# alexklwong/calibrated-backprojection-network

Hardware: AMD Instinct MI355X
Metric: depth-completion frames/sec at 352x1216 (higher is better)
Workload: dtype f32; 1 GPU; KITTI 352x1216, batch 32/GPU, fp32, full KBNet forward in HIP, random xavier weights; frames_per_gpu=32, global_batch=32, height=352, width=1216, n_ranks_seen=1, collective_backend=nccl, gathered_frames=32, launch=HIP graph replay, 2 concurrent sub-batch branch(es)

## Files before the change

### calibrated-backprojection-network_amd/csrc/conv_split.hip

```cpp
#include "conv_common.h"

#ifndef KBN_SPLIT_STRAIGHT
#define KBN_SPLIT_STRAIGHT 1
#endif
#ifndef KBN_SPLIT_PRIO
#define KBN_SPLIT_PRIO 0
#endif

namespace kbn {

typedef _Float16 sph8 __attribute__((ext_vector_type(8)));
typedef _Float16 sph2 __attribute__((ext_vector_type(2)));
typedef float spf16 __attribute__((ext_vector_type(16)));
typedef float spf4 __attribute__((ext_vector_type(4)));
typedef _Float16 sph4 __attribute__((ext_vector_type(4)));

constexpr int SP_TW = 32, SP_CK = 16, SP_MB = 4, SP_TH = 16, SP_THREADS = 512;
constexpr int SP_WEXP = 13;

template <int MODE>
struct SpGeom {
    static constexpr bool UP = MODE == 1, S2 = MODE == 2;
    static constexpr int TH = S2 ? 8 : SP_TH;
    static constexpr int ROWS = UP ? TH / 2 + 2 : (S2 ? 2 * TH + 1 : TH + 2);
    static constexpr int COLS = UP ? SP_TW / 2 + 2 : (S2 ? 2 * SP_TW + 1 : SP_TW + 2), NPIX = ROWS * COLS;
    static constexpr int A_PART = 2 * NPIX * 16, A_BYTES = 2 * A_PART;
    static constexpr int LDS = 2 * A_BYTES;
    static constexpr int PR = (NPIX + 255) / 256;
    static constexpr int NLOADA = PR * 8;
};

struct SplitConvParams {
    const float* src[2];
    long long src_bstride[2];
    int srcC[2];
    int nsrc;
    const float* inv_scale;
    const _Float16* wp;
    float* out;
    long long out_bstride;
    int N, OC, Cin, H, W;
    int sH, sW;
    int tilesX, tilesY, nTilesN, nblocks;
    int act;
    float slope;
    int vec4;
    float prescale;
    float unscale;
    const unsigned* amax[2];
    unsigned* out_amax;
    const _Float16* pair_src;
    long long pair_src_bstride;
    const float* pair_src_scale;
    _Float16* pair_out;
    long long pair_out_bstride;
    float* pair_out_scale;
    const float* l1;
    int tp_x0, tp_tilesY, tp_nblocks;
    int sub0;
    const float* xyz;
    long long xyz_bstride;
    const float* wxyz;
    int ksplit;
    long long ks_stride;
};

__device__ __forceinline__ void sp_split8(const float (&v)[8], float prescale, sph8& h1, sph8& h2) {
    const float prescale_hi = prescale * 2048.f;
#pragma unroll
    for (int k = 0; k < 8; k += 2) {
        const f32x2 a = {v[k], v[k + 1]};
        const sph2 c1 = __builtin_convertvector(a * prescale, sph2);
        const f32x2 f = {(float)c1[0], (float)c1[1]};
        const f32x2 hi = a * prescale_hi;
        const f32x2 r = {__builtin_fmaf(f[0], -2048.f, hi[0]), __builtin_fmaf(f[1], -2048.f, hi[1])};
        const sph2 c2 = __builtin_convertvector(r, sph2);
        h1[k] = c1[0]; h1[k + 1] = c1[1];
        h2[k] = c2[0]; h2[k + 1] = c2[1];
    }
}

__device__ __forceinline__ void sp_act_scale(const SplitConvParams& p, int n, float& prescale, float& unscale) {
    prescale = p.prescale;
    unscale = p.unscale;
    if (p.amax[0]) {
        unsigned b = p.amax[0][n];
        if (p.amax[1]) b = max(b, p.amax[1][n]);
        int k = 14 + 127 - (int)(b >> 23);
        k = k > 100 ? 100 : (k < -100 ? -100 : k);
        prescale = __uint_as_float((unsigned)(127 + k) << 23);
        unscale = __uint_as_float((unsigned)(127 - k) << 23);
    }
}
__device__ __forceinline__ float sp_amax4(float m, const f32x4& v) {
    return fmaxf(fmaxf(m, fmaxf(fin_abs(v[0]), fin_abs(v[1]))), fmaxf(fin_abs(v[2]), fin_abs(v[3])));
}


__device__ __forceinline__ float sp_scale_of_bound(float bound) {
    int k = 14 + 127 - (int)(__float_as_uint(bound) >> 23 & 255u);
    k = k > 100 ? 100 : (k < -100 ? -100 : k);
    return __uint_as_float((unsigned)(127 + k) << 23);
}
__device__ __forceinline__ float sp_pair_out_scale(const SplitConvParams& p, int n) {
    const int nchunks = p.Cin / SP_CK, n0 = p.nsrc > 1 ? p.srcC[0] / SP_CK : nchunks;
    float w0 = 0.f, w1 = 0.f;
    for (int c = 0; c < n0; ++c) w0 += p.l1[c];
    for (int c = n0; c < nchunks; ++c) w1 += p.l1[c];
    float bound = __uint_as_float(p.amax[0][n]) * w0;
    if (p.nsrc > 1) bound += __uint_as_float(p.amax[1][n]) * w1;
    return sp_scale_of_bound(bound);
}
__device__ __forceinline__ void sp_act_scale_of(const SplitConvParams& p, int s, int n, float& prescale, float& unscale) {
// ... 56 lines not shown
__global__ void pack_split_kernel(const float* __restrict__ w, const float* __restrict__ inv_scale, _Float16* __restrict__ packed,
                                  int OC, int Cin, int nchunks, int NT, long long total, int taps, int skip_at, int skip) {
    const long long e = (long long)blockIdx.x * blockDim.x + threadIdx.x;
    if (e >= total) return;
    const int per_chunk = taps * 2 * 2 * NT * 8;
    int r = (int)(e % per_chunk);
    const long long q = e / per_chunk;
    const int chunk = (int)(q % nchunks), nt = (int)(q / nchunks);
    const int tap = r / (2 * 2 * NT * 8); r -= tap * 2 * 2 * NT * 8;
    const int part = r / (2 * NT * 8); r -= part * 2 * NT * 8;
    const int g = r / (NT * 8); r -= g * NT * 8;
    const int n = r >> 3, k = r & 7;
    const int c = chunk * SP_CK + g * 8 + k, oc = nt * NT + n;
    _Float16 h = (_Float16)0.f;
    if (c < Cin && oc < OC) {
        const int cw = c < skip_at ? c : c + skip;
        const float ws = w[((long long)oc * (Cin + skip) + cw) * taps + tap] * (1.f / inv_scale[oc]);
        const _Float16 w1 = (_Float16)ws;
        h = part == 0 ? w1 : (_Float16)((ws - (float)w1) * 2048.f);

    }
    packed[e] = h;
}

__global__ __launch_bounds__(256) void split_l1_kernel(const float* __restrict__ w, float* __restrict__ l1, int OC, int Cin, int taps) {
    __shared__ float red[256];
    const int c = blockIdx.x;
    float m = 0.f;
    for (int oc = threadIdx.x; oc < OC; oc += 256) {
        const float* wp = w + ((long long)oc * Cin + c * SP_CK) * taps;
        float sum = 0.f;
        for (int e = 0; e < SP_CK * taps; ++e) sum += fabsf(wp[e]);
        m = fmaxf(m, sum);
    }
    red[threadIdx.x] = m;
    __syncthreads();
    for (int st = 128; st > 0; st >>= 1) {
        if ((int)threadIdx.x < st) red[threadIdx.x] = fmaxf(red[threadIdx.x], red[threadIdx.x + st]);
        __syncthreads();
    }
    if (threadIdx.x == 0) l1[c] = red[0];
}

template <bool VEC>
__global__ __launch_bounds__(256) void absmax_frames_kernel(const float* __restrict__ x, long long batch_stride, long long per_frame,
                                                            unsigned* __restrict__ slots) {
    const float* xn = x + (long long)blockIdx.y * batch_stride;
    float m = 0.f;
    const long long stride = (long long)gridDim.x * 256;
    if constexpr (VEC) {
        const f32x4* x4 = reinterpret_cast<const f32x4*>(xn);
        const long long n4 = per_frame >> 2;
        long long i = (long long)blockIdx.x * 256 + threadIdx.x;
        for (; i + 3 * stride < n4; i += 4 * stride) {
            const f32x4 a = x4[i], b = x4[i + stride], c = x4[i + 2 * stride], d = x4[i + 3 * stride];
            m = sp_amax4(sp_amax4(sp_amax4(sp_amax4(m, a), b), c), d);
        }
        for (; i < n4; i += stride) m = sp_amax4(m, x4[i]);
        for (long long t = (n4 << 2) + (long long)blockIdx.x * 256 + threadIdx.x; t < per_frame; t += stride) m = fmaxf(m, fin_abs(xn[t]));
    } else {
        for (long long i = (long long)blockIdx.x * 256 + threadIdx.x; i < per_frame; i += stride) m = fmaxf(m, fin_abs(xn[i]));
    }
    absmax_commit(slots + blockIdx.y, m);
}

int absmax_frames_launch(const float* x, long long batch_stride, int n, long long per_frame, unsigned* slots, hipStream_t stream) {
    if (!x || !slots || n < 1 || per_frame < 1) return KBN_ERR_INVALID_ARGUMENT;
    const bool vec = !((reinterpret_cast<uintptr_t>(x) & 15) || (batch_stride & 3));
    const int blocks = (int)std::min<long long>(std::max(1, 2048 / n), (per_frame + 4095) / 4096);
    if (vec) hipLaunchKernelGGL(absmax_frames_kernel<true>, dim3(blocks, n), dim3(256), 0, stream, x, batch_stride, per_frame, slots);
    else hipLaunchKernelGGL(absmax_frames_kernel<false>, dim3(blocks, n), dim3(256), 0, stream, x, batch_stride, per_frame, slots);
    KBN_CHECK_LAUNCH();
    return KBN_OK;
}

template <int N, int NBX>
__device__ __forceinline__ void sp_wait_b(f32x4 (&b)[NBX][2]) {
    static_assert(NBX == 1 || NBX == 2, "one or two 32-filter blocks per wave");
    if constexpr (NBX == 2) asm volatile("s_waitcnt vmcnt(%4)" : "+v"(b[0][0]), "+v"(b[0][1]), "+v"(b[1][0]), "+v"(b[1][1]) : "n"(N));
    else asm volatile("s_waitcnt vmcnt(%2)" : "+v"(b[0][0]), "+v"(b[0][1]) : "n"(N));
}

template <int MODE, int RG, bool APART, bool BLDS, int NBW = 2, bool PIN0 = false, bool POUT = false, bool MIXED = false, bool ONE = false, bool KSPLIT = false>
__global__ __launch_bounds__(SP_THREADS, 1) void conv3x3_split_kernel(const SplitConvParams p) {
    static_assert(!MIXED || (MODE == 0 && BLDS), "transposed tiles: the concat kernel");
    extern __shared__ __attribute__((aligned(16))) unsigned char smem[];
    if (!MIXED || (int)blockIdx.x < p.nblocks) {
        constexpr bool TP = false;
        const int block = blockIdx.x, nblocks = p.nblocks, tilesX = p.tilesX, tilesY = p.tilesY;
#include "conv_split_body.inc"
    } else if constexpr (MIXED) {
        constexpr bool TP = true;
        const int block = (int)blockIdx.x - p.nblocks, nblocks = p.tp_nblocks, tilesX = 1, tilesY = p.tp_tilesY;
#include "conv_split_body.inc"
    }
}

constexpr int UF_NT = 32, UF_ITEMS = 16;
struct UfItem { int ox, s, py, dy, px, dx; };
__host__ __device__ constexpr UfItem uf_item(int it) {
    int ox = it < 4 ? 0 : (it < 12 ? 1 : 2);
    int r = it - (ox == 0 ? 0 : (ox == 1 ? 4 : 12));
    const int ncol = ox == 1 ? 2 : 1;
    const int rowidx = r / ncol, colidx = r % ncol;
    const int s = rowidx == 0 ? 0 : (rowidx < 3 ? 1 : 2);
    const int py = s == 0 ? 0 : (s == 2 ? 1 : rowidx - 1);
    const int px = ox == 0 ? 0 : (ox == 2 ? 1 : colidx);
    return UfItem{ox, s, py, s - py, px, ox - px};
}
__device__ __forceinline__ void uf_taps(int p, int d, int tr, int& k0, int& k1) {
    if (tr) { k0 = p == 0 ? 1 : (d == 0 ? 2 : 0); k1 = (p == 0 && d == 0) ? 0 : k0; return; }
    k0 = (p == 0) ? (d == 0 ? 0 : 1) : (d == 0 ? 0 : 2);
    k1 = (p == 0) ? (d == 0 ? 0 : 2) : (d == 0 ? 1 : 2);
}
__device__ __forceinline__ float uf_fold(const float* w9, int py, int dy, int px, int dx, int tr = 0) {
    int r0, r1, c0, c1;
    uf_taps(py, dy, tr, r0, r1);
    uf_taps(px, dx, tr, c0, c1);
    float acc = 0.f;
    for (int r = r0; r <= r1; ++r) {
        float row = 0.f;
        for (int c = c0; c <= c1; ++c) row += w9[r * 3 + c];
        acc += row;
    }
    return acc;
}

__global__ void uf_scale_kernel(const float* __restrict__ w, float* __restrict__ inv_scale, int OC, int Cin, int tr) {
    const int oc = blockIdx.x;
    __shared__ float red[256];
    float m = 0.f;
    if (oc < OC)
        for (int i = threadIdx.x; i < Cin * UF_ITEMS; i += 256) {
            const int c = i / UF_ITEMS;
            const UfItem t = uf_item(i % UF_ITEMS);
            m = fmaxf(m, fabsf(uf_fold(w + ((long long)oc * Cin + c) * 9, t.py, t.dy, t.px, t.dx, tr)));
        }
    red[threadIdx.x] = m;
    __syncthreads();
    for (int s = 128; s > 0; s >>= 1) {
        if (threadIdx.x < s) red[threadIdx.x] = fmaxf(red[threadIdx.x], red[threadIdx.x + s]);
        __syncthreads();
    }
    if (threadIdx.x == 0) {
        int ex = SP_WEXP;
        if (red[0] > 0.f && red[0] < 3.0e38f) (void)frexpf(red[0], &ex);
        int e = SP_WEXP - ex;
        e = e > 100 ? 100 : (e < -100 ? -100 : e);
        inv_scale[oc] = ldexpf(1.f, -e);
    }
}

__global__ void uf_pack_kernel(const float* __restrict__ w, const float* __restrict__ inv_scale, _Float16* __restrict__ packed,
                               int OC, int Cin, int nchunks, long long total, int tr) {
    const long long e = (long long)blockIdx.x * blockDim.x + threadIdx.x;
    if (e >= total) return;
    constexpr int per_item = 2 * 2 * UF_NT * 8, per_chunk = UF_ITEMS * per_item;
    int r = (int)(e % per_chunk);
    const long long q = e / per_chunk;
    const int chunk = (int)(q % nchunks), nt = (int)(q / nchunks);
    const int item = r / per_item; r -= item * per_item;
    const int part = r / (2 * UF_NT * 8); r -= part * 2 * UF_NT * 8;
    const int g = r / (UF_NT * 8); r -= g * UF_NT * 8;
    const int n = r >> 3, k = r & 7;
    const int c = chunk * SP_CK + g * 8 + k, oc = nt * UF_NT + n;
    _Float16 h = (_Float16)0.f;
    if (c < Cin && oc < OC) {
// ... 944 lines not shown
            if (s != 0 || mode == 1) return KBN_ERR_UNSUPPORTED;
            if (mode == 2 && n_src != 1) return KBN_ERR_UNSUPPORTED;
            if (mode == 0 && (n_src != 2 || a.channels < 2 * SP_CK || srcs[1].kind != KBN_SRC_TENSOR || srcs[1].channels < 2 * SP_CK))
                return KBN_ERR_UNSUPPORTED;
            if (!a.scale || (reinterpret_cast<uintptr_t>(a.data) & 15) || (a.batch_stride & 7) ||
                a.batch_stride < (long long)(a.channels / 8) * 2 * pair_plane_halves(a.src_height, a.src_width))
                return KBN_ERR_INVALID_ARGUMENT;
            if ((long long)a.src_height * a.src_width >= 0x0fffffffLL) return KBN_ERR_UNSUPPORTED;
            p.pair_src = reinterpret_cast<const _Float16*>(a.data); p.pair_src_bstride = a.batch_stride; p.pair_src_scale = a.scale;
        } else {
            p.src[s] = a.data; p.src_bstride[s] = a.batch_stride;
        }
        p.srcC[s] = a.channels;
        cin += a.channels;
    }
    if (p.pair_src && !p.src[0]) { p.src[0] = p.src[1]; p.src_bstride[0] = p.src_bstride[1]; }
    const bool dims_ok = mode == 0 ? (p.sH == height && p.sW == width)
                       : mode != 2 ? (2 * p.sH == height && 2 * p.sW == width)
                                   : (ceil_div(p.sH, 2) == height && ceil_div(p.sW, 2) == width);
    if (!dims_ok) return KBN_ERR_INVALID_ARGUMENT;
    if ((long long)p.sH * p.sW > 0x1fffffffLL || (long long)height * width > 0x1fffffffLL) return KBN_ERR_UNSUPPORTED;
    if (n_src == 1) { p.src[1] = p.src[0]; p.src_bstride[1] = p.src_bstride[0]; p.srcC[1] = 0; }
    p.nsrc = n_src;
    if (srcs[0].absmax && (n_src == 1 || srcs[1].absmax)) { p.amax[0] = srcs[0].absmax; p.amax[1] = n_src > 1 ? srcs[1].absmax : nullptr; }
    else if (p.pair_src && n_src > 1 && srcs[1].absmax) p.amax[1] = srcs[1].absmax;
    p.out_amax = out_absmax;
    const int ntf = split_nt(mode, out_channels, cin);
    p.nTilesN = ceil_div(out_channels, ntf);
    p.inv_scale = static_cast<const float*>(packed_weight);
    p.wp = reinterpret_cast<const _Float16*>(p.inv_scale + p.nTilesN * ntf);
    p.l1 = reinterpret_cast<const float*>(static_cast<const unsigned char*>(packed_weight) +
                                          kbn_conv3x3_split_packed_weight_bytes(out_channels, cin, mode) - (size_t)(cin / SP_CK) * 4);
    if (pair_out) {
        const bool narrow = mode == 3 && uf_narrow(out_channels, cin) && !(knob(KNOB_DEBUG) & 128);
        const bool kernel_ok = (mode == 0) || (mode == 3 && ntf == U64_NT && !uf_narrow(out_channels, cin)) ||
                               (mode == 2 && n_src == 1) || narrow;
        if (!kernel_ok || (!narrow && (out_channels & 7))) return KBN_ERR_UNSUPPORTED;
        const int pair_channels = narrow ? U16_NT : out_channels;
        if (!p.amax[0] || (n_src > 1 && !p.amax[1]) || !pair_out_scale || (reinterpret_cast<uintptr_t>(pair_out) & 15) ||
            (pair_out_batch_stride & 7) || pair_out_batch_stride < (long long)(pair_channels / 8) * 2 * pair_plane_halves(height, width))
            return KBN_ERR_INVALID_ARGUMENT;
        p.pair_out = static_cast<_Float16*>(pair_out); p.pair_out_bstride = pair_out_batch_stride; p.pair_out_scale = pair_out_scale;
    }
    if (p.pair_src && mode == 3 && !(ntf == U64_NT || uf_narrow(out_channels, cin))) return KBN_ERR_UNSUPPORTED;
    if (p.pair_src && mode == 3 && uf_narrow(out_channels, cin) && (srcs[0].channels % U16_CK)) return KBN_ERR_UNSUPPORTED;
    p.out = out; p.out_bstride = out_batch_stride;
    p.N = n; p.OC = out_channels; p.Cin = cin; p.H = height; p.W = width;
    p.tilesX = ceil_div(width, SP_TW); p.tilesY = ceil_div(height, mode == 2 ? SpGeom<2>::TH : SpGeom<0>::TH);
    if (mode == 3) { p.tilesX = ceil_div(p.sW, 32); p.tilesY = ceil_div(p.sH, 16); }
    const long long blocks = (long long)p.tilesX * p.tilesY * n * p.nTilesN;
    if (blocks > 0x7fffffffLL) return KBN_ERR_UNSUPPORTED;
    p.nblocks = (int)blocks;
    p.act = apply_activation ? 1 : 0; p.slope = negative_slope;
    p.prescale = ldexpf(1.f, act_exponent); p.unscale = ldexpf(1.f, -act_exponent);
    p.vec4 = vec4 ? 1 : 0;
    p.ksplit = 1;
    if (ksplit > 1) {
        const bool up64 = mode == 3 && ntf == U64_NT && !uf_narrow(out_channels, cin);
        if ((mode != 0 && mode != 2 && !up64) || p.pair_src || pair_out || !workspace || !out || knob(KNOB_FP16_ONE_TERM)) return KBN_ERR_UNSUPPORTED;
        const int nchunks = cin / SP_CK;
        if (ksplit > nchunks || (long long)(ceil_div(nchunks, ksplit)) * (ksplit - 1) >= nchunks) return KBN_ERR_INVALID_ARGUMENT;
        if (blocks * ksplit > 0x7fffffffLL) return KBN_ERR_UNSUPPORTED;
        const long long per_frame = (long long)out_channels * height * width;
        SplitConvParams q = p;
        q.ksplit = ksplit;
        q.out = workspace; q.out_bstride = per_frame; q.ks_stride = per_frame * n;
        q.out_amax = nullptr; q.act = 0;
        q.vec4 = !((width & 3) || (reinterpret_cast<uintptr_t>(workspace) & 15)) ? 1 : 0;
        q.nblocks = (int)(blocks * ksplit);
        static DeviceOnce ok0, ok2, ok3;
        if (up64) {
            q.tilesX = ceil_div(p.sW, 32); q.tilesY = ceil_div(p.sH, 8);
            const long long b64 = (long long)q.tilesX * q.tilesY * n * p.nTilesN * ksplit;
            if (b64 > 0x7fffffffLL) return KBN_ERR_UNSUPPORTED;
            q.nblocks = (int)b64;
            auto kern = upconv2x_split64_kernel<false, false, false, false, true>;
            if (int r = set_max_dynamic_lds(ok3, reinterpret_cast<const void*>(kern), 160 * 1024)) return r;
            hipLaunchKernelGGL(kern, dim3(q.nblocks), dim3(SP_THREADS), 2 * (2 * 2 * 10 * 34 * 16) + 2 * (8 * 2 * 2 * 64 * 16), (hipStream_t)stream, q);
        } else if (mode == 0) {
            auto kern = conv3x3_split_kernel<0, 8, true, true, 2, false, false, false, false, true>;
            if (int r = set_max_dynamic_lds(ok0, reinterpret_cast<const void*>(kern), 160 * 1024)) return r;
            hipLaunchKernelGGL(kern, dim3(q.nblocks), dim3(SP_THREADS), SpGeom<0>::LDS + 2 * 9 * 2 * 2 * 64 * 16, (hipStream_t)stream, q);
        } else {
            auto kern = conv3x3_split_kernel<2, 2, true, false, 1, false, false, false, false, true>;
            if (int r = set_max_dynamic_lds(ok2, reinterpret_cast<const void*>(kern), 160 * 1024)) return r;
            hipLaunchKernelGGL(kern, dim3(q.nblocks), dim3(SP_THREADS), SpGeom<2>::LDS, (hipStream_t)stream, q);
        }
        KBN_CHECK_LAUNCH();
        const float slope = apply_activation ? negative_slope : 1.f;
        const bool vec = !(per_frame & 3) && !(out_batch_stride & 3) && !((reinterpret_cast<uintptr_t>(out) | reinterpret_cast<uintptr_t>(workspace)) & 15);
        const long long items = vec ? per_frame / 4 : per_frame;
        long long kr = items / (256LL * 512);
        kr = kr < 1 ? 1 : (kr > 8 ? 8 : kr);
        const dim3 grid((unsigned)((items + 256 * kr - 1) / (256 * kr)), (unsigned)n);
        if (vec) hipLaunchKernelGGL(ksplit_reduce_kernel<true>, grid, dim3(256), 0, (hipStream_t)stream, workspace, q.ks_stride, ksplit, out, out_batch_stride, per_frame, slope, out_absmax, (int)kr);
        else hipLaunchKernelGGL(ksplit_reduce_kernel<false>, grid, dim3(256), 0, (hipStream_t)stream, workspace, q.ks_stride, ksplit, out, out_batch_stride, per_frame, slope, out_absmax, (int)kr);
        KBN_CHECK_LAUNCH();
        return KBN_OK;
    }
    const bool one_term = knob(KNOB_FP16_ONE_TERM) != 0;
    auto launch = [&](auto kern, size_t lds, DeviceOnce& once) -> int {
        if (int rc = set_max_dynamic_lds(once, reinterpret_cast<const void*>(kern), 160 * 1024)) return rc;
        hipLaunchKernelGGL(kern, dim3(p.nblocks), dim3(SP_THREADS), lds, (hipStream_t)stream, p);
        return KBN_OK;
    };
    static DeviceOnce o[5];
    int rc;
    if (mode == 3 && uf_narrow(out_channels, cin)) {
        if (knob(KNOB_DEBUG) & 128) {
            static DeviceOnce o8p;
            rc = p.pair_src ? launch(upconv2x_split16_kernel<8, true>, 2 * 2 * 4 * ((18 * 34 + 15) / 16 * 16) * 16, o8p)
                            : launch(upconv2x_split16_kernel<8, false>, 2 * 2 * 4 * ((18 * 34 + 15) / 16 * 16) * 16, o[4]);
        } else {
            p.tilesY = ceil_div(p.sH, 8);
            const long long blocks8 = (long long)p.tilesX * p.tilesY * n * p.nTilesN;
            if (blocks8 > 0x7fffffffLL) return KBN_ERR_UNSUPPORTED;
            p.nblocks = (int)blocks8;
            static DeviceOnce o16, o16p, o16o, o16po;
            auto launch4 = [&](auto kern, DeviceOnce& once) -> int {
                if (int r = set_max_dynamic_lds(once, reinterpret_cast<const void*>(kern), 160 * 1024)) return r;
                hipLaunchKernelGGL(kern, dim3(p.nblocks), dim3(256), 2 * 4 * ((10 * 34 + 15) / 16 * 16) * 16, (hipStream_t)stream, p);
                return KBN_OK;
            };
            if (one_term && p.pair_src && p.pair_out) {
                static DeviceOnce o16po1;
                rc = launch4(upconv2x_split16_kernel<4, true, true, true>, o16po1);
            } else if (p.pair_out) rc = p.pair_src ? launch4(upconv2x_split16_kernel<4, true, true>, o16po) : launch4(upconv2x_split16_kernel<4, false, true>, o16o);
            else rc = p.pair_src ? launch4(upconv2x_split16_kernel<4, true>, o16p) : launch4(upconv2x_split16_kernel<4, false>, o16);
        }
        if (rc != KBN_OK) return rc;
        KBN_CHECK_LAUNCH();
        return KBN_OK;
    }
    if (mode == 3 && ntf == U64_NT) {
        p.tilesX = ceil_div(p.sW, 32); p.tilesY = ceil_div(p.sH, 8);
        const long long blocks64 = (long long)p.tilesX * p.tilesY * n * p.nTilesN;
        if (blocks64 > 0x7fffffffLL) return KBN_ERR_UNSUPPORTED;
        p.nblocks = (int)blocks64;
        constexpr size_t lds64 = 2 * (2 * 2 * 10 * 34 * 16) + 2 * (8 * 2 * 2 * 64 * 16);
        const int wrem = p.sW % 32;
        const bool tp64 = p.sW >= 32 && wrem >= 1 && wrem <= 16 && !(knob(KNOB_DEBUG) & 512);
        if (tp64) {
            p.tilesX = p.sW / 32;
            p.nblocks = p.tilesX * p.tilesY * n * p.nTilesN;
            p.tp_x0 = 32 * p.tilesX;
            p.tp_tilesY = ceil_div(p.sH, 16);
            p.tp_nblocks = p.tp_tilesY * n * p.nTilesN;
        }
        auto launch64 = [&](auto kern, DeviceOnce& once) -> int {
            if (int r = set_max_dynamic_lds(once, reinterpret_cast<const void*>(kern), 160 * 1024)) return r;
            hipLaunchKernelGGL(kern, dim3(p.nblocks + (tp64 ? p.tp_nblocks : 0)), dim3(SP_THREADS), lds64, (hipStream_t)stream, p);
            return KBN_OK;
        };
        auto pick64 = [&](auto one_tag) -> int {
            constexpr bool ONE = decltype(one_tag)::value;
            static DeviceOnce o64[4], o64t[4];
            if (tp64) {
                if (p.pair_src) return p.pair_out ? launch64(upconv2x_split64_kernel<true, true, true, ONE>, o64t[3]) : launch64(upconv2x_split64_kernel<true, false, true, ONE>, o64t[2]);
                return p.pair_out ? launch64(upconv2x_split64_kernel<false, true, true, ONE>, o64t[1]) : launch64(upconv2x_split64_kernel<false, false, true, ONE>, o64t[0]);
            }
            if (p.pair_src) return p.pair_out ? launch64(upconv2x_split64_kernel<true, true, false, ONE>, o64[3]) : launch64(upconv2x_split64_kernel<true, false, false, ONE>, o64[2]);
            return p.pair_out ? launch64(upconv2x_split64_kernel<false, true, false, ONE>, o64[1]) : launch64(upconv2x_split64_kernel<false, false, false, ONE>, o64[0]);
        };
        rc = one_term ? pick64(std::true_type{}) : pick64(std::false_type{});
        if (rc != KBN_OK) return rc;
        KBN_CHECK_LAUNCH();
        return KBN_OK;
    }
    switch (mode) {
        case 0:
            {
                constexpr size_t lds0 = SpGeom<0>::LDS + 2 * 9 * 2 * 2 * 64 * 16;
                const int wrem = width % SP_TW;
                const bool tp = width >= SP_TW && wrem >= 1 && wrem <= 16 && !(knob(KNOB_DEBUG) & 512);
                if (tp) {
                    p.tilesX = width / SP_TW;
                    p.nblocks = p.tilesX * p.tilesY * n * p.nTilesN;
                    p.tp_x0 = SP_TW * p.tilesX;
                    p.tp_tilesY = ceil_div(height, 2 * SpGeom<0>::TH);
                    p.tp_nblocks = p.tp_tilesY * n * p.nTilesN;
                }
                auto launch0 = [&](auto kern, DeviceOnce& once) -> int {
                    if (int r = set_max_dynamic_lds(once, reinterpret_cast<const void*>(kern), 160 * 1024)) return r;
                    hipLaunchKernelGGL(kern, dim3(p.nblocks + (tp ? p.tp_nblocks : 0)), dim3(SP_THREADS), lds0, (hipStream_t)stream, p);
                    return KBN_OK;
                };
                auto pick0 = [&](auto one_tag) -> int {
                    constexpr bool ONE = decltype(one_tag)::value;
                    static DeviceOnce o0p[4], o0t[4];
                    if (tp) {
                        if (p.pair_src) return p.pair_out ? launch0(conv3x3_split_kernel<0, 8, true, true, 2, true, true, true, ONE>, o0t[3])
                                                          : launch0(conv3x3_split_kernel<0, 8, true, true, 2, true, false, true, ONE>, o0t[2]);
                        return p.pair_out ? launch0(conv3x3_split_kernel<0, 8, true, true, 2, false, true, true, ONE>, o0t[1])
                                          : launch0(conv3x3_split_kernel<0, 8, true, true, 2, false, false, true, ONE>, o0t[0]);
                    }
                    if (p.pair_src) return p.pair_out ? launch0(conv3x3_split_kernel<0, 8, true, true, 2, true, true, false, ONE>, o0p[3])
                                                      : launch0(conv3x3_split_kernel<0, 8, true, true, 2, true, false, false, ONE>, o0p[2]);
                    return p.pair_out ? launch0(conv3x3_split_kernel<0, 8, true, true, 2, false, true, false, ONE>, o0p[1])
                                      : launch0(conv3x3_split_kernel<0, 8, true, true, 2, false, false, false, ONE>, o0p[0]);
                };
                rc = one_term ? pick0(std::true_type{}) : pick0(std::false_type{});
            }
            break;
        case 1: return KBN_ERR_UNSUPPORTED;
        case 2:
            {
                auto pick2 = [&](auto one_tag) -> int {
                    constexpr bool ONE = decltype(one_tag)::value;
                    static DeviceOnce o2p[4];
                    if (p.pair_src) return p.pair_out ? launch(conv3x3_split_kernel<2, 2, true, false, 1, true, true, false, ONE>, SpGeom<2>::LDS, o2p[3])
                                                      : launch(conv3x3_split_kernel<2, 2, true, false, 1, true, false, false, ONE>, SpGeom<2>::LDS, o2p[2]);
                    return p.pair_out ? launch(conv3x3_split_kernel<2, 2, true, false, 1, false, true, false, ONE>, SpGeom<2>::LDS, o2p[1])
                                      : launch(conv3x3_split_kernel<2, 2, true, false, 1, false, false, false, ONE>, SpGeom<2>::LDS, o2p[0]);
                };
                rc = one_term ? pick2(std::true_type{}) : pick2(std::false_type{});
            }
            break;
        default:
            rc = launch(upconv2x_split_kernel<true>, 2 * (2 * 2 * 18 * 34 * 16) + 2 * UF_ITEMS * (2 * 2 * UF_NT * 16), o[3]);
            break;
    }
    if (rc != KBN_OK) return rc;
    KBN_CHECK_LAUNCH();
    return KBN_OK;
}


int kbn_conv3x3_split_forward(const kbn_conv_src* srcs, int n_src, const void* packed_weight, float* out,
                              long long out_batch_stride, int n, int out_channels, int height, int width, int mode,
                              int act_exponent, int apply_activation, float negative_slope, unsigned* out_absmax,
                              void* pair_out, long long pair_out_batch_stride, float* pair_out_scale, kbn_stream_t stream) {
    return conv3x3_split_impl(srcs, n_src, packed_weight, out, out_batch_stride, n, out_channels, height, width, mode, act_exponent,
                              apply_activation, negative_slope, out_absmax, pair_out, pair_out_batch_stride, pair_out_scale, 1, nullptr, stream);
}

int kbn_conv3x3_split_forward_ksplit(const kbn_conv_src* srcs, int n_src, const void* packed_weight, float* out,
                                     long long out_batch_stride, int n, int out_channels, int height, int width, int mode,
                                     int act_exponent, int apply_activation, float negative_slope, unsigned* out_absmax,
                                     int ksplit, float* workspace, kbn_stream_t stream) {
    if (ksplit < 1) return KBN_ERR_INVALID_ARGUMENT;
    return conv3x3_split_impl(srcs, n_src, packed_weight, out, out_batch_stride, n, out_channels, height, width, mode, act_exponent,
                              apply_activation, negative_slope, out_absmax, nullptr, 0, nullptr, ksplit, workspace, stream);
}


static size_t c1_panel_bytes(int out_channels, int cin) {
    return (size_t)kbn::ceil_div(out_channels, 128) * (128 * 4 + (size_t)(cin / kbn::SP_CK) * (2 * 2 * 128 * 16));
}

size_t kbn_conv1x1s2_split_packed_weight_bytes(int out_channels, int tensor_channels, int has_xyz) {
    if (out_channels < 1 || tensor_channels < 1 || (tensor_channels % kbn::SP_CK) != 0) return 0;
    return c1_panel_bytes(out_channels, tensor_channels) + (has_xyz ? (size_t)out_channels * 3 * 4 : 0);
}

int kbn_conv1x1s2_split_pack_weight(const float* weight, void* packed, int out_channels, int in_channels, int xyz_offset,
                                    kbn_stream_t stream) {
    using namespace kbn;
    const bool has_xyz = xyz_offset >= 0;
    const int cin = in_channels - (has_xyz ? 3 : 0);
    if (!weight || !packed || (has_xyz && xyz_offset > cin) || kbn_conv1x1s2_split_packed_weight_bytes(out_channels, cin, has_xyz) == 0)
        return KBN_ERR_INVALID_ARGUMENT;
    const int ocpad = ceil_div(out_channels, 128) * 128;
    float* inv = static_cast<float*>(packed);
    _Float16* wp = reinterpret_cast<_Float16*>(inv + ocpad);
    const long long total = (long long)((c1_panel_bytes(out_channels, cin) - (size_t)ocpad * 4) / 2);
    hipLaunchKernelGGL(split_scale_kernel, dim3(ocpad), dim3(256), 0, (hipStream_t)stream, weight, inv, out_channels, in_channels);
    hipLaunchKernelGGL(pack_split_kernel, dim3((unsigned)((total + 255) / 256)), dim3(256), 0, (hipStream_t)stream, weight, inv, wp,
                       out_channels, cin, cin / SP_CK, 128, total, 1, has_xyz ? xyz_offset : cin, has_xyz ? 3 : 0);
    if (has_xyz) {
        float* wxyz = reinterpret_cast<float*>(static_cast<unsigned char*>(packed) + c1_panel_bytes(out_channels, cin));
        hipLaunchKernelGGL(copy_wxyz_kernel, dim3(ceil_div(out_channels * 3, 256)), dim3(256), 0, (hipStream_t)stream, weight, wxyz,
                           out_channels, in_channels, xyz_offset);
    }
    KBN_CHECK_LAUNCH();
    return KBN_OK;
}

int kbn_conv1x1s2_split_forward(const kbn_conv_src* srcs, int n_src, const void* packed_weight, const float* xyz,
                                long long xyz_batch_stride, float* out, long long out_batch_stride, int n, int out_channels,
                                int height, int width, int act_exponent, int apply_activation, float negative_slope,
                                unsigned* out_absmax, kbn_stream_t stream) {
    using namespace kbn;
    if (act_exponent < -60 || act_exponent > 60) return KBN_ERR_INVALID_ARGUMENT;
    if (!srcs || n_src < 1 || n_src > 2 || !packed_weight || !out || n < 1 || out_channels < 1 || height < 1 || width < 1)
        return KBN_ERR_INVALID_ARGUMENT;
    if (knob(KNOB_NO_SPLIT)) return KBN_ERR_UNSUPPORTED;
    SplitConvParams p{};
    int cin = 0;
    for (int s = 0; s < n_src; ++s) {
        const kbn_conv_src& a = srcs[s];
        if (a.kind != KBN_SRC_TENSOR || !a.data || a.channels < 1 || (a.channels % SP_CK) != 0) return KBN_ERR_UNSUPPORTED;
        const bool sub = s == 0 && n_src == 2 && a.src_height == height && a.src_width == width &&
                         (srcs[1].src_height != height || srcs[1].src_width != width);
        if (sub) p.sub0 = 1;
        else {
            if (!p.sH) { p.sH = a.src_height; p.sW = a.src_width; }
// ... 48 lines not shown
```

### calibrated-backprojection-network_amd/csrc/conv_split_body.inc

```
    static_assert(APART, "the two small terms share the scale 2^11 and an accumulator of their own");
    static_assert(!(PIN0 || POUT) || (MODE == 0 && BLDS) || (MODE == 2 && !BLDS), "pair tensors: the concat kernel and the stride-2 kernel");
    using G = SpGeom<MODE>;
    constexpr bool UP = G::UP, S2 = G::S2;
    constexpr int NB = NBW, FG = 8 / RG;
    constexpr int NT = 32 * NB * FG, NPIX = G::NPIX, PR = G::PR, COLS = TP ? 18 : G::COLS;
    static_assert(!TP || NPIX == 34 * 18, "the transposed region has the staged tile's size");
    constexpr int MB = G::TH / RG;
    static_assert(MB == 2 || MB == 4, "groups per chunk must be even (ping-pong A fragments)");
    constexpr int B_TAP = 2 * 2 * NT * 16;
    asm volatile("s_setreg_imm32_b32 hwreg(HW_REG_MODE, 6, 2), 0");
    const int tid = threadIdx.x, lane = tid & 63;
    const int wave = __builtin_amdgcn_readfirstlane(tid >> 6);
    const int rg = wave % RG, fg = wave / RG;
    const int lm = lane & 31, g = lane >> 5;
    int bid = xcd_remap(block, nblocks);
    int ks = 0;
    if constexpr (KSPLIT) { ks = bid % p.ksplit; bid /= p.ksplit; }
    const int nt = bid % p.nTilesN;
    bid /= p.nTilesN;
    const int tx = bid % tilesX;
    bid /= tilesX;
    const int ty = bid % tilesY;
    const int n = bid / tilesY;
    const int oy0 = ty * (TP ? 2 * G::TH : G::TH), ox0 = TP ? p.tp_x0 : tx * SP_TW;
    const int H = p.H, W = p.W, sH = p.sH, sW = p.sW;
    const long long plane = (long long)sH * sW;
    const int nchunks = p.Cin / SP_CK;
    int c_lo = 0, c_hi = nchunks;
    if constexpr (KSPLIT) {
        static_assert(!PIN0 && !POUT && !TP, "the split-K form: fp32 sources in, partial fp32 sums out, whole tiles");
        const int per = (nchunks + p.ksplit - 1) / p.ksplit;
        c_lo = ks * per;
        c_hi = min(nchunks, c_lo + per);
    }
    float prescale, unscale;
    float acc_rescale = 1.f;
    if constexpr (PIN0) {
        const float unscale0 = 1.f / p.pair_src_scale[n];
        prescale = 0.f; unscale = unscale0;
        if (MODE == 0 && p.nsrc > 1) {
            sp_act_scale_of(p, 1, n, prescale, unscale);
            acc_rescale = prescale * unscale0;
            if (!(acc_rescale <= 0x1p60f)) { acc_rescale = 1.f; prescale = p.pair_src_scale[n]; unscale = unscale0; }
        }
    } else sp_act_scale(p, n, prescale, unscale);

    const int kg_st = wave >> 2, t256 = tid & 255;
    int goff[PR], slot[PR];
#pragma unroll
    for (int u = 0; u < PR; ++u) {
        const int pix = u * 256 + t256;
        const int r = pix / COLS, c = pix - r * COLS;
        const int Y = (UP ? (oy0 >> 1) : (S2 ? 2 * oy0 : oy0)) - 1 + r, X = (UP ? (ox0 >> 1) : (S2 ? 2 * ox0 : ox0)) - 1 + c;
        goff[u] = (pix < NPIX && Y >= 0 && Y < sH && X >= 0 && X < sW) ? (Y * sW + X) * 4 : -1;
        slot[u] = S2 ? r * COLS + ((c & 1) ? (COLS + 1) / 2 + (c >> 1) : (c >> 1)) : pix;
    }
    const _Float16* wp_nt = p.wp + (long long)nt * nchunks * (9 * B_TAP / 2);

    float va[PR][8];
    auto load_chunk = [&](int chunk) {
        int c = chunk * SP_CK, s = 0;
        if (p.nsrc > 1 && c >= p.srcC[0]) { c -= p.srcC[0]; s = 1; }
        const float* base = p.src[s] + (long long)n * p.src_bstride[s] + (long long)(c + kg_st * 8) * plane;
#pragma unroll
        for (int u = 0; u < PR; ++u) {
            const unsigned voff = goff[u] < 0 ? 0u : (unsigned)goff[u];
#pragma unroll
            for (int k = 0; k < 8; ++k) {
                const float* sb = base + (long long)k * plane;
                asm volatile("global_load_dword %0, %1, %2" : "=v"(va[u][k]) : "v"(voff), "s"(sb) : "memory");
            }
        }
    };
    auto store_round = [&](int buf, int u) {
        unsigned char* A = smem + buf * G::A_BYTES + kg_st * NPIX * 16;
#pragma unroll
        for (int k = 0; k < 8; ++k) asm volatile("" : "+v"(va[u][k]));
        const int pix = u * 256 + t256;
        if (pix < NPIX) {
            float v[8];
#pragma unroll
            for (int k = 0; k < 8; ++k) v[k] = goff[u] >= 0 ? va[u][k] : 0.f;
            sph8 h1, h2;
            sp_split8(v, prescale, h1, h2);
            *reinterpret_cast<sph8*>(A + slot[u] * 16) = h1;
            if (!ONE) *reinterpret_cast<sph8*>(A + G::A_PART + slot[u] * 16) = h2;
        }
    };
    const unsigned boff = (unsigned)((g * NT + fg * 32 * NB + lm) * 16);
    auto load_b = [&](f32x4 (&b)[NB][2], int chunk, int tap) {
        const unsigned char* base = reinterpret_cast<const unsigned char*>(wp_nt + ((long long)chunk * 9 + tap) * (B_TAP / 2));
#pragma unroll
        for (int nb = 0; nb < NB; ++nb)
#pragma unroll
            for (int t = 0; t < 2; ++t) {
                const unsigned char* sb = base + (t * 2 * NT + nb * 32) * 16;
                asm volatile("global_load_dwordx4 %0, %1, %2" : "=v"(b[nb][t]) : "v"(boff), "s"(sb) : "memory");
            }
    };

    spf16 acc[MB][NB], lo[APART ? MB : 1][NB];
#pragma unroll
    for (int mb = 0; mb < MB; ++mb)
#pragma unroll
        for (int nb = 0; nb < NB; ++nb)
#pragma unroll
            for (int i = 0; i < 16; ++i) {
                acc[mb][nb][i] = 0.f;
                if (APART) lo[mb][nb][i] = 0.f;
            }

    constexpr int GM = 1, GPT = MB / GM, NGROUP = 9 * GPT;
    const unsigned char* aptr[3];
#pragma unroll
    for (int kx = 0; kx < 3; ++kx)
        aptr[kx] = TP ? smem + (g * NPIX + (2 * MB * rg + (lm >> 4)) * COLS + (lm & 15) + kx) * 16
                      : smem + (g * NPIX + (UP ? MB / 2 : (S2 ? 2 * MB : MB)) * rg * COLS +
                                (UP ? ((lm + kx + 1) >> 1) : (S2 ? (kx == 1 ? (COLS + 1) / 2 + lm : lm + (kx >> 1)) : lm + kx))) * 16;
    auto load_a = [&](sph8 (&a)[GM][2], int abuf_off, int grp) {
        const int tap = grp / GPT, mb0 = (grp % GPT) * GM;
        const int ky = tap / 3, kx = tap % 3;
#pragma unroll
        for (int m = 0; m < GM; ++m) {
            const int r = UP ? ((mb0 + m + ky + 1) >> 1) : ((S2 || TP) ? 2 * (mb0 + m) + ky : mb0 + m + ky);
#pragma unroll
            for (int t = 0; t < 2; ++t)
                a[m][t] = *reinterpret_cast<const sph8*>(aptr[kx] + abuf_off + t * G::A_PART + r * COLS * 16);
        }
    };
    auto mfma_group = [&](auto chk_tag, const sph8 (&a)[GM][2], const sph8 (&b)[NB][2], int grp) {
        constexpr bool CHK = decltype(chk_tag)::value;
        const bool nb0_live = nt * NT + fg * 32 * NB < p.OC, nb1_live = nt * NT + fg * 32 * NB + 32 < p.OC;
        const int mb0 = (grp % GPT) * GM;
        constexpr int TA[3] = {0, 0, 1}, TBP[3] = {0, 1, 0};
        constexpr int NTERM = ONE ? 1 : 3;
#pragma unroll
        for (int t = 0; t < NTERM; ++t)
#pragma unroll
            for (int m = 0; m < GM; ++m)
#pragma unroll
                for (int nb = 0; nb < NB; ++nb) {
                    if (CHK && oy0 + (TP ? 2 : 1) * (MB * rg + mb0 + m) >= H) continue;
                    if (CHK && !(nb == 0 ? nb0_live : nb1_live)) continue;
                    spf16& c = (APART && t > 0) ? lo[mb0 + m][nb] : acc[mb0 + m][nb];
                    c = POUT ? __builtin_amdgcn_mfma_f32_32x32x16_f16(b[nb][TBP[t]], a[m][TA[t]], c, 0, 0, 0)
                             : __builtin_amdgcn_mfma_f32_32x32x16_f16(a[m][TA[t]], b[nb][TBP[t]], c, 0, 0, 0);
                }
    };
    const bool padded_tile = !KBN_SPLIT_STRAIGHT || oy0 + (TP ? 2 * G::TH : G::TH) > H || (nt + 1) * NT - 32 >= p.OC;

    f32x4 bq[3][NB][2];
    constexpr int AD = 1;
    static_assert(NGROUP % (AD + 1) == 0, "the fragment rotation must close over a chunk");
    sph8 aq[AD + 1][GM][2];
    if constexpr (BLDS) {
        constexpr int B_CHUNK = 9 * B_TAP;
        const unsigned lds0 = __builtin_amdgcn_readfirstlane(lds_addr(reinterpret_cast<const float*>(smem)));
        auto stage_b = [&](int bbuf, int chunk) {
            const float* src = reinterpret_cast<const float*>(wp_nt + (long long)chunk * (B_CHUNK / 2));
            const unsigned dst = lds0 + (unsigned)(2 * G::A_BYTES + bbuf * B_CHUNK);
            constexpr int n4 = B_CHUNK / 16;
// ... 31 lines not shown
            }
        };
        auto body = [&](int c_in, auto next_tag, auto chk_tag) __attribute__((always_inline)) {

            const int c = PIN0 ? __builtin_amdgcn_readfirstlane(c_in) : c_in;
            constexpr int NEXT = decltype(next_tag)::value;
            constexpr bool MORE = NEXT != 0;
            const int abuf = (c & 1) * G::A_BYTES;
            const unsigned char* B = bptr + (c & 1) * B_CHUNK;
            if (MORE) {
                stage_b((c & 1) ^ 1, c + 1);
                if constexpr (NEXT == 2) dma_chunk((c & 1) ^ 1, c + 1);
                else load_chunk(c + 1);
            }
            load_a(aq[0], abuf, 0);
            sph8 bw[NB][2];
#pragma unroll
            for (int grp = 0; grp < NGROUP; ++grp) {
                const int tap = grp / GPT, gi = grp % GPT;
                sph8 (&ac)[GM][2] = aq[grp % (AD + 1)];
                if (grp + AD < NGROUP) load_a(aq[(grp + AD) % (AD + 1)], abuf, grp + AD);
                if (gi == 0) {
#pragma unroll
                    for (int nb = 0; nb < NB; ++nb) {
                        bw[nb][0] = *reinterpret_cast<const sph8*>(B + tap * B_TAP + nb * 32 * 16);
                        bw[nb][1] = *reinterpret_cast<const sph8*>(B + tap * B_TAP + (2 * NT + nb * 32) * 16);
                    }
                }
                if (MORE && grp == 5 * GPT) asm volatile("s_waitcnt vmcnt(0)" ::: "memory");
                __builtin_amdgcn_sched_barrier(0x8);
#if KBN_SPLIT_PRIO == 1
                __builtin_amdgcn_s_setprio(1);
#endif
                mfma_group(chk_tag, ac, bw, grp);
#if KBN_SPLIT_PRIO == 1
                __builtin_amdgcn_s_setprio(0);
#endif
                __builtin_amdgcn_sched_barrier(0x8);
                if (NEXT == 1 && tap >= 5) {
                    const int u = (tap - 5) * GPT + gi;
                    if (u < PR) store_round((c & 1) ^ 1, u);
                }
            }
            __syncthreads();
        };
        if constexpr (PIN0) dma_chunk(0, 0);
        else load_chunk(c_lo);
        stage_b(c_lo & 1, c_lo);
        asm volatile("s_waitcnt vmcnt(0)" ::: "memory");
        if constexpr (!PIN0) {
#pragma unroll
            for (int u = 0; u < PR; ++u) store_round(c_lo & 1, u);
        }
        __syncthreads();
#if KBN_SPLIT_PRIO == 2
        if (wave >= 4) __builtin_amdgcn_s_setprio(1);
#endif
        using Next0 = std::integral_constant<int, 0>;
        using Next1 = std::integral_constant<int, 1>;
        using Next2 = std::integral_constant<int, 2>;
        auto k_loop = [&](auto chk_tag) {
            if constexpr (PIN0) {
                const int n0 = p.srcC[0] / SP_CK;
                int c = 0;
                do body(c, Next2{}, chk_tag); while (++c < n0 - 1);
                body(n0 - 1, Next1{}, chk_tag);
#pragma unroll
                for (int mb = 0; mb < MB; ++mb)
#pragma unroll
                    for (int nb = 0; nb < NB; ++nb)
#pragma unroll
                        for (int i = 0; i < 16; ++i) { acc[mb][nb][i] *= acc_rescale; lo[mb][nb][i] *= acc_rescale; }
                c = n0;
                do body(c, Next1{}, chk_tag); while (++c < nchunks - 1);
                body(nchunks - 1, Next0{}, chk_tag);
            } else {
                for (int c = c_lo; c + 1 < c_hi; ++c) body(c, Next1{}, chk_tag);
                body(c_hi - 1, Next0{}, chk_tag);
            }
        };
        if (padded_tile) k_loop(std::true_type{});
        else k_loop(std::false_type{});
    } else {
    constexpr int NR2 = (NPIX + 63) / 64, NDMA2 = 4 * NR2, DPW2 = NDMA2 / 8;
    static_assert(!PIN0 || NDMA2 % 8 == 0, "the same number of DMAs in every wave (the vmcnt arithmetic counts them)");
    const unsigned lds0s = __builtin_amdgcn_readfirstlane(lds_addr(reinterpret_cast<const float*>(smem)));
    unsigned dvoff2[PIN0 ? DPW2 : 1];
    if constexpr (PIN0) {
#pragma unroll
        for (int i = 0; i < DPW2; ++i) {
            const int q = ((wave + 8 * i) % NR2) * 64 + lane;
            const int r = q / COLS, sc = q - r * COLS;
            const int cc = S2 ? (sc < (COLS + 1) / 2 ? 2 * sc : 2 * (sc - (COLS + 1) / 2) + 1) : sc;
            const int Y = (S2 ? 2 * oy0 : oy0) - 1 + r, X = (S2 ? 2 * ox0 : ox0) - 1 + cc;
            dvoff2[i] = (q < NPIX && Y >= 0 && Y < sH && X >= 0 && X < sW) ? (unsigned)(Y * sW + X) * 16u : (unsigned)(sH * sW) * 16u;
        }
    }
    const long long pplane2 = pair_plane_halves(sH, sW);
    auto dma_chunk2 = [&](int buf, int chunk) __attribute__((always_inline)) {

        const _Float16* pn = p.pair_src + (long long)n * p.pair_src_bstride + (long long)(2 * chunk) * 2 * pplane2;
#pragma unroll
        for (int i = 0; i < DPW2; ++i) {
            const int id = wave + 8 * i, plane = id / NR2, j = id - plane * NR2;
            const int t = plane >> 1, kgl = plane & 1;
            const unsigned long long mask = (j == NR2 - 1 && (NPIX & 63)) ? ((1ull << (NPIX & 63)) - 1) : ~0ull;
            lds_dma16_sm(reinterpret_cast<const float*>(pn + (long long)(kgl * 2 + t) * pplane2), dvoff2[i],
                         lds0s + (unsigned)(buf * G::A_BYTES + t * G::A_PART + (kgl * NPIX + j * 64) * 16), mask);
        }
    };
    auto chunk_body = [&](int c, auto more_tag, auto chk_tag) {
        constexpr bool MORE = decltype(more_tag)::value;
        constexpr int NA = MORE ? (PIN0 ? DPW2 : G::NLOADA) : 0, NBL = 2 * NB;
        const int abuf = (c & 1) * G::A_BYTES;
#pragma unroll
        for (int d = 0; d < AD; ++d) load_a(aq[d], abuf, d);
        sph8 bw[NB][2];
#pragma unroll
        for (int grp = 0; grp < NGROUP; ++grp) {
            const int tap = grp / GPT, gi = grp % GPT;
            f32x4 (&bc)[NB][2] = bq[tap % 3];
            f32x4 (&bn)[NB][2] = bq[(tap + 2) % 3];
            sph8 (&ac)[GM][2] = aq[grp % (AD + 1)];
            if (grp + AD < NGROUP) load_a(aq[(grp + AD) % (AD + 1)], abuf, grp + AD);
            if (gi == 0) {
                if (tap + 2 < 9) load_b(bn, c, tap + 2);
                else if (MORE) load_b(bn, c + 1, tap + 2 - 9);
                if (tap == 0 && MORE) {
                    if constexpr (PIN0) dma_chunk2((c & 1) ^ 1, c + 1);
                    else load_chunk(c + 1);
                }
                if (tap <= 2) sp_wait_b<2 * NBL + NA>(bc);
                else if (tap < 7 || MORE) sp_wait_b<2 * NBL>(bc);
                else if (tap == 7) sp_wait_b<NBL>(bc);
                else sp_wait_b<0>(bc);
#pragma unroll
                for (int nb = 0; nb < NB; ++nb) {
                    bw[nb][0] = __builtin_bit_cast(sph8, bc[nb][0]);
                    bw[nb][1] = __builtin_bit_cast(sph8, bc[nb][1]);
                }
            }
            __builtin_amdgcn_sched_barrier(0);
            mfma_group(chk_tag, ac, bw, grp);
            __builtin_amdgcn_sched_barrier(0);
            static_assert(5 * GPT >= PR, "taps 4-8 hold the staging rounds");
            if (!PIN0 && MORE && tap >= 4) {
                const int u = (tap - 4) * GPT + gi;
                if (u < PR) store_round((c & 1) ^ 1, u);
            }
        }
        __syncthreads();
    };

    if constexpr (PIN0) dma_chunk2(0, 0);
    else load_chunk(c_lo);
    load_b(bq[0], c_lo, 0);
    load_b(bq[1], c_lo, 1);
    asm volatile("s_waitcnt vmcnt(0)" ::: "memory");
    if constexpr (!PIN0) {
#pragma unroll
        for (int u = 0; u < PR; ++u) store_round(c_lo & 1, u);
    }
    __syncthreads();
    auto k_loop = [&](auto chk_tag) {
        for (int c = c_lo; c + 1 < c_hi; ++c) chunk_body(c, std::true_type{}, chk_tag);
        chunk_body(c_hi - 1, std::false_type{}, chk_tag);
    };
    if (padded_tile) k_loop(std::true_type{});
    else k_loop(std::false_type{});
    }

    const float slope = (p.act && !KSPLIT) ? p.slope : 1.f;
    float amax = 0.f;
    if constexpr (POUT) {
        const float ps_out = sp_pair_out_scale(p, n);
        const long long oph = pair_plane_halves(H, W);
        _Float16* const pn = p.pair_out + (long long)n * p.pair_out_bstride;
        if (tid == 0) p.pair_out_scale[n] = ps_out;
        if (tx == 0 && ty == 0 && wave == 0 && lane < NT / 4) {
            const int kgz = nt * (NT / 8) + (lane >> 1);
            if (kgz * 8 < p.OC)
                *reinterpret_cast<f32x4*>(pn + (long long)(kgz * 2 + (lane & 1)) * oph + (long long)H * W * 8) = (f32x4){0.f, 0.f, 0.f, 0.f};
        }
        const int X = TP ? ox0 + (lm & 15) : ox0 + lm;
#pragma unroll
        for (int nb = 0; nb < NB; ++nb)
#pragma unroll
// ... 83 lines not shown
```

Baseline: 2992 frames/s.

## Shrink stride-2 conv tiles to 4 rows with 256-thread workgroups, two per CU

The stride-2 split conv kernel now uses 4-row output tiles (configurable) with 256-thread workgroups, and launch bounds allow two resident workgroups per CU. Thread and wave counts, the staging loops and the DMA distribution are generalised to the new wave count. The aim is more independent workgroups per CU and finer tiles, so latency hides better and load balances better on the stride-2 layers. In exchange the halo overhead per tile grows, and the register budget per thread shrinks because of the two-per-CU bound.

```diff
diff --git a/calibrated-backprojection-network_amd/csrc/conv_split.hip b/calibrated-backprojection-network_amd/csrc/conv_split.hip
--- a/calibrated-backprojection-network_amd/csrc/conv_split.hip
+++ b/calibrated-backprojection-network_amd/csrc/conv_split.hip
@@ -18,17 +18,27 @@
 constexpr int SP_TW = 32, SP_CK = 16, SP_MB = 4, SP_TH = 16, SP_THREADS = 512;
 constexpr int SP_WEXP = 13;
 
+#ifndef KBN_S2_TH
+#define KBN_S2_TH 4
+#endif
+static_assert(KBN_S2_TH == 4 || KBN_S2_TH == 8, "stride-2 tiles: 4 or 8 output rows");
+
 template <int MODE>
 struct SpGeom {
     static constexpr bool UP = MODE == 1, S2 = MODE == 2;
-    static constexpr int TH = S2 ? 8 : SP_TH;
+    static constexpr int TH = S2 ? KBN_S2_TH : SP_TH;
+    static constexpr int THREADS = S2 ? 64 * KBN_S2_TH : SP_THREADS;
+    static constexpr int NW = THREADS / 64, HALF = THREADS / 2;
+    static constexpr int WG_PER_CU = SP_THREADS / THREADS;
     static constexpr int ROWS = UP ? TH / 2 + 2 : (S2 ? 2 * TH + 1 : TH + 2);
     static constexpr int COLS = UP ? SP_TW / 2 + 2 : (S2 ? 2 * SP_TW + 1 : SP_TW + 2), NPIX = ROWS * COLS;
     static constexpr int A_PART = 2 * NPIX * 16, A_BYTES = 2 * A_PART;
     static constexpr int LDS = 2 * A_BYTES;
-    static constexpr int PR = (NPIX + 255) / 256;
+    static constexpr int PR = (NPIX + HALF - 1) / HALF;
     static constexpr int NLOADA = PR * 8;
+    static_assert(LDS * WG_PER_CU <= 160 * 1024, "the resident workgroups' tiles fit in a CU's LDS");
 };
+constexpr int SP_S2_RG = KBN_S2_TH / SP_MB;
 
 struct SplitConvParams {
     const float* src[2];
@@ -251,7 +261,7 @@
 }
 
 template <int MODE, int RG, bool APART, bool BLDS, int NBW = 2, bool PIN0 = false, bool POUT = false, bool MIXED = false, bool ONE = false, bool KSPLIT = false>
-__global__ __launch_bounds__(SP_THREADS, 1) void conv3x3_split_kernel(const SplitConvParams p) {
+__global__ __launch_bounds__(SpGeom<MODE>::THREADS, SpGeom<MODE>::WG_PER_CU) void conv3x3_split_kernel(const SplitConvParams p) {
     static_assert(!MIXED || (MODE == 0 && BLDS), "transposed tiles: the concat kernel");
     extern __shared__ __attribute__((aligned(16))) unsigned char smem[];
     if (!MIXED || (int)blockIdx.x < p.nblocks) {
@@ -1362,9 +1372,9 @@
             if (int r = set_max_dynamic_lds(ok0, reinterpret_cast<const void*>(kern), 160 * 1024)) return r;
             hipLaunchKernelGGL(kern, dim3(q.nblocks), dim3(SP_THREADS), SpGeom<0>::LDS + 2 * 9 * 2 * 2 * 64 * 16, (hipStream_t)stream, q);
         } else {
-            auto kern = conv3x3_split_kernel<2, 2, true, false, 1, false, false, false, false, true>;
+            auto kern = conv3x3_split_kernel<2, SP_S2_RG, true, false, 1, false, false, false, false, true>;
             if (int r = set_max_dynamic_lds(ok2, reinterpret_cast<const void*>(kern), 160 * 1024)) return r;
-            hipLaunchKernelGGL(kern, dim3(q.nblocks), dim3(SP_THREADS), SpGeom<2>::LDS, (hipStream_t)stream, q);
+            hipLaunchKernelGGL(kern, dim3(q.nblocks), dim3(SpGeom<2>::THREADS), SpGeom<2>::LDS, (hipStream_t)stream, q);
         }
         KBN_CHECK_LAUNCH();
         const float slope = apply_activation ? negative_slope : 1.f;
@@ -1379,9 +1389,9 @@
         return KBN_OK;
     }
     const bool one_term = knob(KNOB_FP16_ONE_TERM) != 0;
-    auto launch = [&](auto kern, size_t lds, DeviceOnce& once) -> int {
+    auto launch = [&](auto kern, size_t lds, DeviceOnce& once, int threads = SP_THREADS) -> int {
         if (int rc = set_max_dynamic_lds(once, reinterpret_cast<const void*>(kern), 160 * 1024)) return rc;
-        hipLaunchKernelGGL(kern, dim3(p.nblocks), dim3(SP_THREADS), lds, (hipStream_t)stream, p);
+        hipLaunchKernelGGL(kern, dim3(p.nblocks), dim3(threads), lds, (hipStream_t)stream, p);
         return KBN_OK;
     };
     static DeviceOnce o[5];
@@ -1485,13 +1495,15 @@
         case 1: return KBN_ERR_UNSUPPORTED;
         case 2:
             {
+                constexpr int RG2 = SP_S2_RG, T2 = SpGeom<2>::THREADS;
+                constexpr size_t L2 = SpGeom<2>::LDS;
                 auto pick2 = [&](auto one_tag) -> int {
                     constexpr bool ONE = decltype(one_tag)::value;
                     static DeviceOnce o2p[4];
-                    if (p.pair_src) return p.pair_out ? launch(conv3x3_split_kernel<2, 2, true, false, 1, true, true, false, ONE>, SpGeom<2>::LDS, o2p[3])
-                                                      : launch(conv3x3_split_kernel<2, 2, true, false, 1, true, false, false, ONE>, SpGeom<2>::LDS, o2p[2]);
-                    return p.pair_out ? launch(conv3x3_split_kernel<2, 2, true, false, 1, false, true, false, ONE>, SpGeom<2>::LDS, o2p[1])
-                                      : launch(conv3x3_split_kernel<2, 2, true, false, 1, false, false, false, ONE>, SpGeom<2>::LDS, o2p[0]);
+                    if (p.pair_src) return p.pair_out ? launch(conv3x3_split_kernel<2, RG2, true, false, 1, true, true, false, ONE>, L2, o2p[3], T2)
+                                                      : launch(conv3x3_split_kernel<2, RG2, true, false, 1, true, false, false, ONE>, L2, o2p[2], T2);
+                    return p.pair_out ? launch(conv3x3_split_kernel<2, RG2, true, false, 1, false, true, false, ONE>, L2, o2p[1], T2)
+                                      : launch(conv3x3_split_kernel<2, RG2, true, false, 1, false, false, false, ONE>, L2, o2p[0], T2);
                 };
                 rc = one_term ? pick2(std::true_type{}) : pick2(std::false_type{});
             }
diff --git a/calibrated-backprojection-network_amd/csrc/conv_split_body.inc b/calibrated-backprojection-network_amd/csrc/conv_split_body.inc
--- a/calibrated-backprojection-network_amd/csrc/conv_split_body.inc
+++ b/calibrated-backprojection-network_amd/csrc/conv_split_body.inc
@@ -2,7 +2,7 @@
     static_assert(!(PIN0 || POUT) || (MODE == 0 && BLDS) || (MODE == 2 && !BLDS), "pair tensors: the concat kernel and the stride-2 kernel");
     using G = SpGeom<MODE>;
     constexpr bool UP = G::UP, S2 = G::S2;
-    constexpr int NB = NBW, FG = 8 / RG;
+    constexpr int NB = NBW, FG = G::NW / RG;
     constexpr int NT = 32 * NB * FG, NPIX = G::NPIX, PR = G::PR, COLS = TP ? 18 : G::COLS;
     static_assert(!TP || NPIX == 34 * 18, "the transposed region has the staged tile's size");
     constexpr int MB = G::TH / RG;
@@ -45,11 +45,11 @@
         }
     } else sp_act_scale(p, n, prescale, unscale);
 
-    const int kg_st = wave >> 2, t256 = tid & 255;
+    const int kg_st = wave / (G::NW / 2), thalf = tid & (G::HALF - 1);
     int goff[PR], slot[PR];
 #pragma unroll
     for (int u = 0; u < PR; ++u) {
-        const int pix = u * 256 + t256;
+        const int pix = u * G::HALF + thalf;
         const int r = pix / COLS, c = pix - r * COLS;
         const int Y = (UP ? (oy0 >> 1) : (S2 ? 2 * oy0 : oy0)) - 1 + r, X = (UP ? (ox0 >> 1) : (S2 ? 2 * ox0 : ox0)) - 1 + c;
         goff[u] = (pix < NPIX && Y >= 0 && Y < sH && X >= 0 && X < sW) ? (Y * sW + X) * 4 : -1;
@@ -76,7 +76,7 @@
         unsigned char* A = smem + buf * G::A_BYTES + kg_st * NPIX * 16;
 #pragma unroll
         for (int k = 0; k < 8; ++k) asm volatile("" : "+v"(va[u][k]));
-        const int pix = u * 256 + t256;
+        const int pix = u * G::HALF + thalf;
         if (pix < NPIX) {
             float v[8];
 #pragma unroll
@@ -274,14 +274,14 @@
         if (padded_tile) k_loop(std::true_type{});
         else k_loop(std::false_type{});
     } else {
-    constexpr int NR2 = (NPIX + 63) / 64, NDMA2 = 4 * NR2, DPW2 = NDMA2 / 8;
-    static_assert(!PIN0 || NDMA2 % 8 == 0, "the same number of DMAs in every wave (the vmcnt arithmetic counts them)");
+    constexpr int NR2 = (NPIX + 63) / 64, NDMA2 = 4 * NR2, DPW2 = NDMA2 / G::NW;
+    static_assert(!PIN0 || NDMA2 % G::NW == 0, "the same number of DMAs in every wave (the vmcnt arithmetic counts them)");
     const unsigned lds0s = __builtin_amdgcn_readfirstlane(lds_addr(reinterpret_cast<const float*>(smem)));
     unsigned dvoff2[PIN0 ? DPW2 : 1];
     if constexpr (PIN0) {
 #pragma unroll
         for (int i = 0; i < DPW2; ++i) {
-            const int q = ((wave + 8 * i) % NR2) * 64 + lane;
+            const int q = ((wave + G::NW * i) % NR2) * 64 + lane;
             const int r = q / COLS, sc = q - r * COLS;
             const int cc = S2 ? (sc < (COLS + 1) / 2 ? 2 * sc : 2 * (sc - (COLS + 1) / 2) + 1) : sc;
             const int Y = (S2 ? 2 * oy0 : oy0) - 1 + r, X = (S2 ? 2 * ox0 : ox0) - 1 + cc;
@@ -294,7 +294,7 @@
         const _Float16* pn = p.pair_src + (long long)n * p.pair_src_bstride + (long long)(2 * chunk) * 2 * pplane2;
 #pragma unroll
         for (int i = 0; i < DPW2; ++i) {
-            const int id = wave + 8 * i, plane = id / NR2, j = id - plane * NR2;
+            const int id = wave + G::NW * i, plane = id / NR2, j = id - plane * NR2;
             const int t = plane >> 1, kgl = plane & 1;
             const unsigned long long mask = (j == NR2 - 1 && (NPIX & 63)) ? ((1ull << (NPIX & 63)) - 1) : ~0ull;
             lds_dma16_sm(reinterpret_cast<const float*>(pn + (long long)(kgl * 2 + t) * pplane2), dvoff2[i],
```

Result: no change. 2979 frames/s, median of 2 (-0.4%).
